# zeropoolnetwork/fawkes-crypto

Measured on AMD Instinct MI355X. Metric: Groth16 proofs/sec + MSM scalar-muls/sec, BN254, 2^25 constraints (33552553 rows = 99.99 % of the 2^25 domain), higher is better.
Workload: dtype u32

## Files before the change

fawkes-crypto_amd/csrc/msm.hip:

```cpp
#include "common.hpp"
#include <algorithm>
#include <string.h>
#include <type_traits>

namespace fk {

static constexpr uint32_t SEG_MAX = 4096, SEG_MIN = 256;
static constexpr uint32_t SORT_THREADS = 256;

struct MsmPlan {
    size_t n;
    uint32_t c, W, B;
    uint32_t cb, wide;
    uint32_t nchunks;
    size_t chunk;
    uint32_t cap, cap_top;
    uint32_t L, T, nblk;
    uint32_t LB, nhi, nlo;
};
#ifndef FK_S2_TILE
#define FK_S2_TILE 8192
#endif
static constexpr uint32_t S2_TILE = FK_S2_TILE;
static constexpr uint32_t S2_EPT = S2_TILE / 1024;
#ifndef FK_S1_TILE
#define FK_S1_TILE 8192
#endif
static constexpr uint32_t S1_TILE = FK_S1_TILE;
#ifndef FK_S2_MAX_HI
#define FK_S2_MAX_HI 1024
#endif
static constexpr uint32_t S2_MAX_HI = FK_S2_MAX_HI;

static MsmPlan make_plan(size_t n, unsigned forced_c, bool merged = false) {
    MsmPlan p{};
    p.n = n;
    const size_t nd = n ? n : 1;
    uint32_t lg = 0; while (((size_t)1 << (lg + 1)) <= nd + nd / 2) lg++;
    static const int t_small = tune("FK_MSM_C_SMALL", 17), t_delta = tune("FK_MSM_C_DELTA", 5), t_sig = tune("FK_MSM_CAP_SIGMA", 6), t_pre_dc = tune("FK_MSM_PRE_DC", 3);
    uint32_t c = forced_c ? forced_c : (lg >= 22 ? lg - t_delta : (lg >= 18 ? (uint32_t)t_small : (lg >= 6 ? lg - 2 : 4)));
    if (merged && !forced_c) c = (uint32_t)std::max(2, (int)c + t_pre_dc);
    if (c < 2) c = 2;
    static const uint32_t t_cmax = (uint32_t)std::min(tune("FK_MSM_C_MAX", 22), S2_MAX_HI >= 2048 ? 24 : 22);
    if (c > t_cmax) c = t_cmax;
    p.c = c;
    p.W = (255 + c - 1) / c;
    p.cb = 255 / p.W;
    p.wide = 255 - p.cb * p.W;
    if (p.wide == 0) { p.cb -= 1; p.wide = p.W; }
    c = p.cb + 1;
    p.c = c;
    p.B = 1u << (c - 1);
    size_t chunk = (n + 255) / 256;
    if (chunk < 16384) chunk = 16384;
    p.chunk = chunk;
    p.nchunks = (uint32_t)((n + chunk - 1) / chunk);
    size_t mean = nd >> (p.wide < p.W ? p.cb - 1 : p.cb);
    p.cap = (uint32_t)std::min<size_t>(2 * mean + 64, 1u << 30);
    if (t_sig > 0) { uint32_t sq = 1; while ((size_t)sq * sq < mean) sq++; p.cap = (uint32_t)std::min<size_t>(mean + (size_t)t_sig * sq + 8, 1u << 30); }
    p.cap_top = p.cap;
    static const int t_redl = tune("FK_MSM_RED_L", 0);
    p.L = p.B >= (1u << 18) ? 64 : (p.B >= (1u << 17) ? p.B / 2048 : (p.B >= 8192 ? p.B / 4096 : 1));
    if (t_redl > 0 && (uint32_t)t_redl <= p.B) p.L = (uint32_t)t_redl;
    static const int t_redl_m = tune("FK_MSM_RED_L_MERGED", 0);
    if (merged) {
        if (p.B <= (1u << 19)) p.L = std::min<uint32_t>(p.L, 8);
        else if (p.B <= (1u << 20)) p.L = std::min<uint32_t>(p.L, 16);
        if (t_redl_m > 0 && (uint32_t)t_redl_m <= p.B) p.L = (uint32_t)t_redl_m;
    }
    p.T = p.B / p.L;
    p.nblk = (p.T + 255) / 256;
    static const int t_lb = std::min(12, std::max(10, tune("FK_MSM_LB", 10)));
    p.LB = (c - 1) < (uint32_t)t_lb ? (c - 1) : (uint32_t)t_lb;
    while ((p.B >> p.LB) > S2_MAX_HI) p.LB++;
    p.nlo = 1u << p.LB;
    p.nhi = p.B >> p.LB;
    return p;
}

__global__ __launch_bounds__(256) void msm_digits_kernel(const Fr *scalars, size_t n, uint32_t cb, uint32_t wide, uint32_t W, uint32_t *digits) {
    const size_t half = (n + 1) / 2;
    const size_t i0 = (size_t)blockIdx.x * blockDim.x + threadIdx.x;
    if (i0 >= half) return;
    const size_t i1 = i0 + half;
    const bool has1 = i1 < n;
    Fr in[2];
    in[0] = scalars[i0];
    in[1] = scalars[has1 ? i1 : i0];
#pragma unroll
    for (int u = 0; u < 2; u++) {
        if (u == 1 && !has1) break;
        const size_t i = u ? i1 : i0;
        Fr s = Fr::from_mont(in[u]);
        uint32_t carry = 0;
        for (uint32_t w = 0; w < W; w++) {
            const uint32_t cw = cb + (w < wide ? 1 : 0);
            const uint32_t o = w * cb + (w < wide ? w : wide), limb = o >> 5, sh = o & 31;
            const uint32_t B = 1u << (cw - 1), mask = (1u << cw) - 1;
            uint32_t lo = limb < 8 ? s.v[limb] : 0, hi = limb + 1 < 8 ? s.v[limb + 1] : 0;
            uint32_t raw = (uint32_t)((((uint64_t)hi << 32) | lo) >> sh) & mask;
            raw += carry;
            uint32_t d, neg;
            if (raw > B) { d = (1u << cw) - raw; neg = 1; carry = 1; } else { d = raw; neg = 0; carry = 0; }
            digits[(size_t)w * n + i] = d | (neg << 31);
        }
    }
}

struct OverEntry { uint32_t g, size; };

static __device__ __forceinline__ uint32_t block_excl_scan_1024(uint32_t v, uint32_t *wsum, uint32_t *total) {
    const uint32_t lane = threadIdx.x & 63, wv = threadIdx.x >> 6;
    uint32_t incl = v;
#pragma unroll
    for (int off = 1; off < 64; off <<= 1) { const uint32_t t = (uint32_t)__shfl_up((int)incl, off, 64); if (lane >= (uint32_t)off) incl += t; }
    if (lane == 63) wsum[wv] = incl;
    __syncthreads();
    uint32_t base = 0, all = 0;
#pragma unroll
    for (uint32_t w = 0; w < 16; w++) { const uint32_t x = wsum[w]; all += x; if (w < wv) base += x; }
    __syncthreads();
    *total = all;
    return base + incl - v;
}

struct MsmDyn {
    uint32_t cap, n_over, seg, n_tasks, n_obs, error, pad0, pad1;
    uint32_t hist[16];
    unsigned long long adds;
};
static constexpr uint32_t OVER_MAX = 4096;

static __device__ __forceinline__ void over_append(bool take, uint32_t g, uint32_t size, OverEntry *over, MsmDyn *dyn) {
    const unsigned long long m = __ballot(take);
    if (!m) return;
    const uint32_t lane = threadIdx.x & 63, leader = (uint32_t)__ffsll((long long)m) - 1;
    uint32_t base = 0;
    if (lane == leader) base = atomicAdd(&dyn->n_over, (uint32_t)__popcll(m));
    base = (uint32_t)__shfl((int)base, (int)leader, 64);
    if (take) {
        const uint32_t k = base + (uint32_t)__popcll(m & ((1ull << lane) - 1));
        if (k < OVER_MAX) { over[k].g = g; over[k].size = size; } else dyn->error = 1;
    }
}

__global__ __launch_bounds__(SORT_THREADS) void s2_hist1_kernel(const uint32_t *digits, size_t n, size_t chunk, uint32_t nchunks,
                                                                 uint32_t LB, uint32_t nhi, uint32_t *cnt1) {
    extern __shared__ uint32_t hist[];
    const uint32_t ch = blockIdx.x, w = blockIdx.y;
    for (uint32_t b = threadIdx.x; b < nhi; b += blockDim.x) hist[b] = 0;
    __syncthreads();
    const size_t lo = (size_t)ch * chunk, hi = lo + chunk < n ? lo + chunk : n;
    const uint32_t *dg = digits + (size_t)w * n;
    for (size_t i = lo + threadIdx.x; i < hi; i += (size_t)blockDim.x * 8) {
        uint32_t d[8];
#pragma unroll
        for (int u = 0; u < 8; u++) { const size_t k = i + (size_t)u * blockDim.x; d[u] = k < hi ? (dg[k] & 0x7fffffffu) : 0; }
#pragma unroll
        for (int u = 0; u < 8; u++) if (d[u]) atomicAdd(&hist[(d[u] - 1) >> LB], 1u);
    }
    __syncthreads();
    uint32_t *out = cnt1 + ((size_t)w * nchunks + ch) * nhi;
    for (uint32_t b = threadIdx.x; b < nhi; b += blockDim.x) out[b] = hist[b];
}

__global__ __launch_bounds__(1024) void s2_prefix1_kernel(uint32_t *cnt1, uint32_t nchunks, uint32_t nhi, uint32_t *seg_size, uint32_t *seg_start,
                                                           uint32_t *seg_tiles) {
    extern __shared__ uint32_t ssz[];
    const uint32_t w = blockIdx.x;
    for (uint32_t h = threadIdx.x; h < nhi; h += blockDim.x) {
        uint32_t run = 0;
        for (uint32_t ch = 0; ch < nchunks; ch++) {
            uint32_t *p = cnt1 + ((size_t)w * nchunks + ch) * nhi + h;
            const uint32_t v = *p; *p = run; run += v;
        }
        ssz[h] = run;
    }
    __syncthreads();
    __shared__ uint32_t part[1024];
    const uint32_t t = threadIdx.x;
    const uint32_t v0 = 2 * t < nhi ? ssz[2 * t] : 0, v1 = 2 * t + 1 < nhi ? ssz[2 * t + 1] : 0;
    part[t] = v0 + v1;
    __syncthreads();
    for (uint32_t off = 1; off < 1024; off <<= 1) {
        const uint32_t x = t >= off ? part[t - off] : 0;
        __syncthreads();
        part[t] += x;
        __syncthreads();
    }
    const uint32_t base = part[t] - (v0 + v1);
    if (2 * t < nhi) { const size_t g = (size_t)w * nhi + 2 * t; seg_size[g] = v0; seg_start[g] = base; seg_tiles[g] = (v0 + S2_TILE - 1) / S2_TILE; }
    if (2 * t + 1 < nhi) { const size_t g = (size_t)w * nhi + 2 * t + 1; seg_size[g] = v1; seg_start[g] = base + v0; seg_tiles[g] = (v1 + S2_TILE - 1) / S2_TILE; }
}

__global__ __launch_bounds__(1024) void s2_tile_prefix_kernel(const uint32_t *seg_tiles, uint32_t nseg, uint32_t *tile_start) {
    __shared__ uint32_t part[1024];
    const uint32_t t = threadIdx.x, per = (nseg + 1023) / 1024;
    const uint32_t lo = t * per, hi = lo + per < nseg ? lo + per : nseg;
    uint32_t sum = 0;
    for (uint32_t s = lo; s < hi; s++) sum += seg_tiles[s];
    part[t] = sum;
    __syncthreads();
    for (uint32_t off = 1; off < 1024; off <<= 1) {
        const uint32_t v = t >= off ? part[t - off] : 0;
        __syncthreads();
        part[t] += v;
        __syncthreads();
    }
    uint32_t run = part[t] - sum;
    for (uint32_t s = lo; s < hi; s++) { tile_start[s] = run; run += seg_tiles[s]; }
    if (t == 1023) tile_start[nseg] = part[1023];
}

static __device__ __forceinline__ uint32_t s2_find_segment(const uint32_t *tile_start, uint32_t nseg, uint32_t t) {
    uint32_t lo = 0, hi = nseg;
    while (hi - lo > 1) { const uint32_t mid = (lo + hi) >> 1; if (tile_start[mid] <= t) lo = mid; else hi = mid; }
    return lo;
}

__global__ __launch_bounds__(256) void s2_hist2_kernel(const uint16_t *tmp_lo, size_t n, uint32_t nhi, uint32_t nlo, const uint32_t *tile_start,
                                                        uint32_t nseg, const uint32_t *seg_start, const uint32_t *seg_size, uint32_t *cnt2) {
    extern __shared__ uint32_t hist[];
    const uint32_t tile = blockIdx.x;
    if (tile >= tile_start[nseg]) return;
    const uint32_t sgm = s2_find_segment(tile_start, nseg, tile), w = sgm / nhi, t = tile - tile_start[sgm];
    for (uint32_t b = threadIdx.x; b < nlo; b += 256) hist[b] = 0;
    __syncthreads();
    const uint32_t size = seg_size[sgm], lo = t * S2_TILE, hi = lo + S2_TILE < size ? lo + S2_TILE : size;
    const uint16_t *src = tmp_lo + (size_t)w * n + seg_start[sgm];
    for (uint32_t k = lo + threadIdx.x; k < hi; k += 256 * 8) {
        uint32_t v[8];
#pragma unroll
        for (uint32_t u = 0; u < 8; u++) { const uint32_t kk = k + u * 256; v[u] = kk < hi ? src[kk] : 0xffffffffu; }
#pragma unroll
        for (uint32_t u = 0; u < 8; u++) if (v[u] != 0xffffffffu) atomicAdd(&hist[v[u]], 1u);
    }
    __syncthreads();
    for (uint32_t b = threadIdx.x; b < nlo; b += 256) cnt2[(size_t)tile * nlo + b] = hist[b];
}

static constexpr uint32_t P2_MAX = 32;
__global__ __launch_bounds__(256) void s2_prefix2_kernel(uint32_t *cnt2, uint32_t nseg, uint32_t nhi, uint32_t nlo, uint32_t B, const uint32_t *tile_start,
                                                          const uint32_t *seg_start, uint32_t cap0, uint32_t *totals, uint32_t *starts, MsmDyn *dyn) {
    __shared__ uint32_t sh_hist[16];
    const uint32_t lane = threadIdx.x & 63, sgm = blockIdx.x * 4 + (threadIdx.x >> 6);
    if (threadIdx.x < 16) sh_hist[threadIdx.x] = 0;
    __syncthreads();
    if (sgm < nseg) {
        const uint32_t w = sgm / nhi, h = sgm % nhi, t0 = tile_start[sgm], t1 = tile_start[sgm + 1];
        uint32_t carry = seg_start[sgm];
        for (uint32_t b0 = 0; b0 < nlo; b0 += 64 * P2_MAX) {
            const uint32_t per = (nlo - b0 + 63) / 64 < P2_MAX ? (nlo - b0 + 63) / 64 : P2_MAX;
            uint32_t run[P2_MAX];
#pragma unroll
            for (uint32_t i = 0; i < P2_MAX; i++) run[i] = 0;
            for (uint32_t t = t0; t < t1; t++) {
                uint32_t *row = cnt2 + (size_t)t * nlo + b0;
// ... 27 lines not shown
    __syncthreads();
    if (threadIdx.x < 16 && sh_hist[threadIdx.x]) atomicAdd(&dyn->hist[threadIdx.x], sh_hist[threadIdx.x]);
}

__global__ void msm_cap_kernel(MsmDyn *dyn, uint32_t cap0, uint32_t many) {
    if (threadIdx.x || blockIdx.x) return;
    uint32_t above[17]; above[16] = 0;
    for (int k = 15; k >= 0; k--) above[k] = above[k + 1] + dyn->hist[k];
    uint32_t k = 0;
    while (k < 15 && above[k] > many && ((unsigned long long)cap0 << k) < (1ull << 20)) k++;
    const unsigned long long c = (unsigned long long)cap0 << k;
    dyn->cap = c < (1ull << 30) ? (uint32_t)c : (1u << 30);
    dyn->n_over = 0; dyn->seg = 0; dyn->n_tasks = 0; dyn->n_obs = 0; dyn->error = 0; dyn->adds = 0;
}

__global__ __launch_bounds__(256) void msm_over_list_kernel(const uint32_t *totals, size_t WB, OverEntry *over, MsmDyn *dyn) {
    const size_t g = (size_t)blockIdx.x * blockDim.x + threadIdx.x;
    const uint32_t sz = g < WB ? totals[g] : 0;
    over_append(g < WB && sz > dyn->cap, (uint32_t)g, sz, over, dyn);
}

template <uint32_t MAXLO>
__global__ __launch_bounds__(1024) void s2_scatter2_kernel(const uint32_t *tmp_idx, const uint16_t *tmp_lo, size_t n, uint32_t nhi, uint32_t nlo, uint32_t B,
                                                            const uint32_t *tile_start, uint32_t nseg, const uint32_t *seg_start, const uint32_t *seg_size,
                                                            const uint32_t *cnt2, const uint32_t *starts, uint32_t *sorted) {
    constexpr uint32_t BPL = MAXLO / 1024;
    __shared__ uint32_t lcnt[MAXLO];
    __shared__ uint32_t wsum[16];
    __shared__ uint32_t gbase[MAXLO];
    __shared__ uint32_t stage_idx[S2_TILE];
    __shared__ uint16_t stage_lo[S2_TILE];
    const uint32_t tile = blockIdx.x, tid = threadIdx.x;
    if (tile >= tile_start[nseg]) return;
    const uint32_t sgm = s2_find_segment(tile_start, nseg, tile), w = sgm / nhi, h = sgm % nhi, t = tile - tile_start[sgm];
#pragma unroll
    for (uint32_t i = 0; i < BPL; i++) {
        const uint32_t b = tid + i * 1024;
        lcnt[b] = 0;
        gbase[b] = b < nlo ? starts[(size_t)w * B + (size_t)h * nlo + b] + cnt2[(size_t)tile * nlo + b] : 0;
    }
    __syncthreads();
    const uint32_t size = seg_size[sgm], lo = t * S2_TILE, cnt = (lo + S2_TILE < size ? lo + S2_TILE : size) - lo;
    const size_t base = (size_t)w * n + seg_start[sgm] + lo;
    uint32_t e_idx[S2_EPT], e_lo[S2_EPT], e_rank[S2_EPT];
#pragma unroll
    for (uint32_t j = 0; j < S2_EPT; j++) {
        const uint32_t k = tid + j * 1024;
        if (k < cnt) { e_idx[j] = tmp_idx[base + k]; e_lo[j] = tmp_lo[base + k]; e_rank[j] = atomicAdd(&lcnt[e_lo[j]], 1u); }
    }
    __syncthreads();
    uint32_t c[BPL], mine = 0;
#pragma unroll
    for (uint32_t i = 0; i < BPL; i++) { c[i] = lcnt[tid * BPL + i]; mine += c[i]; }
    uint32_t all_;
    uint32_t excl = block_excl_scan_1024(mine, wsum, &all_);
#pragma unroll
    for (uint32_t i = 0; i < BPL; i++) { lcnt[tid * BPL + i] = excl; excl += c[i]; }
    __syncthreads();
#pragma unroll
    for (uint32_t j = 0; j < S2_EPT; j++) {
        const uint32_t k = tid + j * 1024;
        if (k < cnt) { const uint32_t q = lcnt[e_lo[j]] + e_rank[j]; stage_idx[q] = e_idx[j]; stage_lo[q] = (uint16_t)e_lo[j]; }
    }
    __syncthreads();
    uint32_t *out = sorted + (size_t)w * n;
    for (uint32_t q = tid; q < cnt; q += 1024) {
        const uint32_t b = stage_lo[q];
        out[gbase[b] + (q - lcnt[b])] = stage_idx[q];
    }
}

__global__ __launch_bounds__(1024) void s2_scatter1_n1024_kernel(const uint32_t *digits, size_t n, size_t chunk, uint32_t nchunks, uint32_t LB,
                                                                  uint32_t nhi, const uint32_t *cnt1, const uint32_t *seg_start, uint32_t *tmp_idx,
                                                                  uint16_t *tmp_lo) {
    constexpr uint32_t NT = 1024;
    constexpr uint32_t BPL = S2_MAX_HI / NT;
    constexpr uint32_t EPT = S1_TILE / NT;
    constexpr bool PREFETCH = EPT <= 16;
    __shared__ uint32_t cursor[S2_MAX_HI];
    __shared__ uint32_t lcnt[S2_MAX_HI];
    __shared__ uint32_t lexc[S2_MAX_HI];
    __shared__ uint32_t part[16];
    __shared__ uint32_t stage_idx[S1_TILE];
    __shared__ uint16_t stage_lo[S1_TILE];
    __shared__ uint16_t stage_bin[S1_TILE];
    const uint32_t ch = blockIdx.x, w = blockIdx.y, tid = threadIdx.x;
    const uint32_t *cnt = cnt1 + ((size_t)w * nchunks + ch) * nhi;
    for (uint32_t b = tid; b < S2_MAX_HI; b += NT) cursor[b] = b < nhi ? seg_start[(size_t)w * nhi + b] + cnt[b] : 0;
    const size_t c_lo = (size_t)ch * chunk, c_hi = c_lo + chunk < n ? c_lo + chunk : n;
    const uint32_t *dg = digits + (size_t)w * n;
    const uint32_t lomask = (1u << LB) - 1;
    uint32_t *oidx = tmp_idx + (size_t)w * n;
    uint16_t *olo = tmp_lo + (size_t)w * n;
    uint32_t d[PREFETCH ? EPT : 1], dn[PREFETCH ? EPT : 1];
    if (PREFETCH && c_lo < c_hi) {
        const uint32_t cnt0 = (uint32_t)(c_hi - c_lo < S1_TILE ? c_hi - c_lo : S1_TILE);
#pragma unroll
        for (uint32_t j = 0; j < EPT; j++) { const uint32_t k = tid + j * NT; d[j] = k < cnt0 ? dg[c_lo + k] : 0; }
    }
    for (size_t sub = c_lo; sub < c_hi; sub += S1_TILE) {
        const uint32_t cntt = (uint32_t)(c_hi - sub < S1_TILE ? c_hi - sub : S1_TILE);
        const uint32_t *src = dg + sub;
        for (uint32_t b = tid; b < S2_MAX_HI; b += NT) lcnt[b] = 0;
        __syncthreads();
        if (PREFETCH) {
#pragma unroll
            for (uint32_t j = 0; j < EPT; j++) { const uint32_t bkt = d[j] & 0x7fffffffu; if (bkt) atomicAdd(&lcnt[(bkt - 1) >> LB], 1u); }
        } else {
#pragma unroll 8
            for (uint32_t k = tid; k < cntt; k += NT) {
                const uint32_t bkt = src[k] & 0x7fffffffu;
                if (bkt) atomicAdd(&lcnt[(bkt - 1) >> LB], 1u);
            }
        }
        __syncthreads();
        uint32_t c[BPL], mine = 0;
#pragma unroll
        for (uint32_t i = 0; i < BPL; i++) { c[i] = lcnt[tid * BPL + i]; mine += c[i]; }
        uint32_t total;
        uint32_t ex = block_excl_scan_1024(mine, part, &total);
#pragma unroll
        for (uint32_t i = 0; i < BPL; i++) { lexc[tid * BPL + i] = ex; ex += c[i]; }
        __syncthreads();
        if (PREFETCH) {
#pragma unroll
            for (uint32_t j = 0; j < EPT; j++) {
                const uint32_t bkt = d[j] & 0x7fffffffu;
                if (bkt) {
                    const uint32_t bin = (bkt - 1) >> LB, q = atomicAdd(&lexc[bin], 1u);
                    stage_idx[q] = (uint32_t)(sub + tid + j * NT) | (d[j] & 0x80000000u); stage_lo[q] = (uint16_t)((bkt - 1) & lomask); stage_bin[q] = (uint16_t)bin;
                }
            }
            const size_t nxt = sub + S1_TILE;
            const uint32_t cntn = nxt < c_hi ? (uint32_t)(c_hi - nxt < S1_TILE ? c_hi - nxt : S1_TILE) : 0;
#pragma unroll
            for (uint32_t j = 0; j < EPT; j++) { const uint32_t k = tid + j * NT; dn[j] = k < cntn ? dg[nxt + k] : 0; }
        } else {
#pragma unroll 8
            for (uint32_t k = tid; k < cntt; k += NT) {
                const uint32_t dd = src[k], bkt = dd & 0x7fffffffu;
                if (bkt) {
                    const uint32_t bin = (bkt - 1) >> LB, q = atomicAdd(&lexc[bin], 1u);
                    stage_idx[q] = (uint32_t)(sub + k) | (dd & 0x80000000u); stage_lo[q] = (uint16_t)((bkt - 1) & lomask); stage_bin[q] = (uint16_t)bin;
                }
            }
        }
        __syncthreads();
#pragma unroll 1
        for (uint32_t q = tid; q < total; q += NT) {
            const uint32_t bn = stage_bin[q];
            const uint32_t dst = cursor[bn] + (q - (lexc[bn] - lcnt[bn]));
            oidx[dst] = stage_idx[q];
            olo[dst] = stage_lo[q];
        }
        __syncthreads();
        for (uint32_t b = tid; b < S2_MAX_HI; b += NT) cursor[b] += lcnt[b];
        if (PREFETCH) {
#pragma unroll
            for (uint32_t j = 0; j < EPT; j++) d[j] = dn[j];
        }
        __syncthreads();
    }
}

static constexpr uint32_t SIZE_BINS = 1024;
static __device__ __forceinline__ uint32_t size_class(uint32_t size, uint32_t cap) {
    const uint32_t s = size < cap ? size : cap;
    if (s < 768) return (SIZE_BINS - 1) - s;
    const uint32_t span = cap > 768 ? cap - 768 : 1;
    return 255u - (uint32_t)(((uint64_t)(s - 768) * 255u) / span);
}
static __device__ __forceinline__ unsigned long long wave_sum_u64(unsigned long long v) {
#pragma unroll
    for (int off = 32; off >= 1; off >>= 1) v += (unsigned long long)__shfl_down((long long)v, off, 64);
    return v;
}
static __device__ __forceinline__ uint32_t dyn_cap(const MsmDyn *dyn, uint32_t mult) {
    const unsigned long long c = (unsigned long long)dyn->cap * mult;
    return c < (1ull << 30) ? (uint32_t)c : (1u << 30);
}
__global__ __launch_bounds__(256) void msm_size_hist_kernel(const uint32_t *totals, size_t WB, const MsmDyn *dyn, uint32_t mult, uint32_t *bins, unsigned long long *adds) {
    __shared__ uint32_t sh[SIZE_BINS];
    const uint32_t cap = dyn_cap(dyn, mult);
    for (uint32_t i = threadIdx.x; i < SIZE_BINS; i += 256) sh[i] = 0;
    __syncthreads();
    unsigned long long mine = 0;
    for (size_t g = (size_t)blockIdx.x * 256 + threadIdx.x; g < WB; g += (size_t)gridDim.x * 256) {
        const uint32_t t = totals[g];
        atomicAdd(&sh[size_class(t, cap)], 1u);
        if (t) mine += (t < cap ? t : cap) - 1;
    }
    __syncthreads();
    for (uint32_t i = threadIdx.x; i < SIZE_BINS; i += 256) if (sh[i]) atomicAdd(&bins[i], sh[i]);
    if (adds) { mine = wave_sum_u64(mine); if ((threadIdx.x & 63) == 0 && mine) atomicAdd(adds, mine); }
}
__global__ __launch_bounds__(SIZE_BINS) void msm_size_scan_kernel(uint32_t *bins) {
    __shared__ uint32_t sh[SIZE_BINS];
    const uint32_t t = threadIdx.x, v = bins[t];
    sh[t] = v;
    __syncthreads();
    for (uint32_t off = 1; off < SIZE_BINS; off <<= 1) {
        uint32_t x = t >= off ? sh[t - off] : 0;
        __syncthreads();
        sh[t] += x;
        __syncthreads();
    }
    bins[t] = sh[t] - v;
}
__global__ __launch_bounds__(1024) void msm_size_scatter_kernel(const uint32_t *totals, size_t WB, const MsmDyn *dyn, uint32_t mult, uint32_t *cursor, uint32_t *perm) {
    __shared__ uint32_t cnt[SIZE_BINS];
    __shared__ uint32_t base[SIZE_BINS];
    const uint32_t cap = dyn_cap(dyn, mult);
    const size_t g = (size_t)blockIdx.x * 1024 + threadIdx.x;
    cnt[threadIdx.x] = 0;
    __syncthreads();
    uint32_t cls = 0, rank = 0;
    if (g < WB) { cls = size_class(totals[g], cap); rank = atomicAdd(&cnt[cls], 1u); }
    __syncthreads();
    if (cnt[threadIdx.x]) base[threadIdx.x] = atomicAdd(&cursor[threadIdx.x], cnt[threadIdx.x]);
    __syncthreads();
    if (g < WB) perm[base[cls] + rank] = (uint32_t)g;
}

template <class T>
static __device__ __forceinline__ T shfl_down_obj(const T &v, int off) {
    static_assert(sizeof(T) % 4 == 0, "word sized");
    T r;
    const uint32_t *s = reinterpret_cast<const uint32_t *>(&v);
    uint32_t *d = reinterpret_cast<uint32_t *>(&r);
#pragma unroll
    for (unsigned i = 0; i < sizeof(T) / 4; i++) d[i] = (uint32_t)__shfl_down((int)s[i], off, 64);
    return r;
}

template <class F>
static __device__ __forceinline__ void wave_reduce(Xyzz<F> &acc) {
#pragma unroll 1
    for (int off = 32; off >= 1; off >>= 1) {
        Xyzz<F> o = shfl_down_obj(acc, off);
// ... 308 lines not shown
    return FK_OK;
}

static int pinned_reserve(fk_ctx *ctx, void **p, size_t *cap, size_t bytes, size_t pad) {
    if (bytes + pad <= *cap) return FK_OK;
    if (*p) { FK_HIP(ctx, hipHostFree(*p)); *p = nullptr; *cap = 0; }
    FK_HIP(ctx, hipHostMalloc(p, bytes + (bytes >> 2) + pad, hipHostMallocDefault));
    *cap = bytes + (bytes >> 2) + pad;
    return FK_OK;
}

template <class F>
struct MsmJob {
    fk_ctx *ctx;
    MsmPlan p;
    MsmLane *ln;
    MsmTail *tl;
    const Affine<F> *bases, *lev;
    const Fr *scalars;
    size_t n, WB, max_tasks, max_tiles, wp_bytes;
    uint32_t WR;
    bool merged, have_sort;
    MsmDyn *dyn;
    uint32_t *digits, *sorted, *totals, *starts, *perm;
    Task *tasks;
    OverBucket *obs;
    Xyzz<F> *winparts;
};

template <class F>
static int msm_reserve(MsmJob<F> &j) {
    fk_ctx *ctx = j.ctx;
    const MsmPlan &p = j.p;
    MsmLane &ln = *j.ln;
    MsmTail &tl = *j.tl;
    const size_t n = j.n, WB = j.WB = (size_t)p.W * p.B;
    j.WR = j.merged ? 1 : p.W;
    j.wp_bytes = (size_t)j.WR * sizeof(Xyzz<F>);
    const size_t wp_dev_bytes = (size_t)j.WR * (p.nblk + 1) * sizeof(Xyzz<F>);
    const size_t max_tasks = j.max_tasks = std::max<size_t>(2048, (size_t)p.W * n / SEG_MAX) + OVER_MAX + 64;
    const uint32_t nseg = p.W * p.nhi;
    const size_t max_tiles = j.max_tiles = (size_t)p.W * ((n + S2_TILE - 1) / S2_TILE) + nseg + 1;
    struct Need { DevBuf *b; size_t bytes; };
    const Need needs[] = {
        {&ln.digits, (size_t)p.W * n * 4}, {&ln.sorted, (size_t)p.W * n * 4}, {&ln.totals, WB * 4}, {&ln.starts, WB * 4},
        {&ln.perm, WB * 4 + SIZE_BINS * 4}, {&ln.overlist, OVER_MAX * sizeof(OverEntry) + sizeof(MsmDyn) + 64}, {j.have_sort ? &ln.buckets2 : &ln.buckets, WB * sizeof(Xyzz<F>)},
        {&ln.tasktab, max_tasks * sizeof(Task) + OVER_MAX * sizeof(OverBucket) + 64}, {&ln.partials, max_tasks * sizeof(Xyzz<F>)},
        {&ln.s2_cnt1, (size_t)p.W * p.nchunks * p.nhi * 4}, {&ln.s2_seg, ((size_t)nseg * 4 + 2) * 4}, {&ln.s2_cnt2, max_tiles * p.nlo * 4},
        {&ln.s2_tmp_idx, (size_t)p.W * n * 4}, {&ln.s2_tmp_lo, (size_t)p.W * n * 2}};
    bool grow = false;
    for (const Need &nd : needs) grow = grow || nd.bytes > nd.b->cap;
    if (grow) {
        FK_HIP(ctx, hipStreamSynchronize(ln.st));
        for (const Need &nd : needs) FK_HIP(ctx, nd.b->reserve(nd.bytes));
        if (!j.have_sort) ln.last_sort_scalars = nullptr;
    }
    FK_HIP(ctx, tl.d_wp.reserve(wp_dev_bytes));
    FK_TRY(pinned_reserve(ctx, &tl.h_wp, &tl.h_cap, j.wp_bytes, 16));
    j.dyn = (MsmDyn *)((char *)ln.overlist.p + OVER_MAX * sizeof(OverEntry));
    j.tasks = ln.tasktab.as<Task>();
    j.obs = (OverBucket *)((char *)ln.tasktab.p + ((max_tasks * sizeof(Task) + 15) & ~(size_t)15));
    j.digits = ln.digits.as<uint32_t>(); j.sorted = ln.sorted.as<uint32_t>();
    j.totals = ln.totals.as<uint32_t>(); j.starts = ln.starts.as<uint32_t>();
    j.winparts = tl.d_wp.as<Xyzz<F>>();
    j.perm = ln.perm.as<uint32_t>();
    return FK_OK;
}

static void launch_scatter2(const MsmPlan &p, uint32_t n_tiles, hipStream_t st, const uint32_t *tmp_idx, const uint16_t *tmp_lo, size_t n, const uint32_t *tile_start, uint32_t nseg,
                            const uint32_t *seg_start, const uint32_t *seg_size, const uint32_t *cnt2, const uint32_t *starts, uint32_t *sorted) {
    const auto kernel = p.nlo <= 1024 ? s2_scatter2_kernel<1024> : (p.nlo <= 2048 ? s2_scatter2_kernel<2048> : s2_scatter2_kernel<4096>);
    hipLaunchKernelGGL(kernel, dim3(n_tiles), dim3(1024), 0, st, tmp_idx, tmp_lo, n, p.nhi, p.nlo, p.B, tile_start, nseg, seg_start, seg_size, cnt2, starts, sorted);
}

template <class F>
static int queue_sort(const MsmJob<F> &j) {
    fk_ctx *ctx = j.ctx;
    const MsmPlan &p = j.p;
    MsmLane &ln = *j.ln;
    hipStream_t st = ln.st;
    const size_t n = j.n;
    const uint32_t nseg = p.W * p.nhi;
    ln.last_sort_scalars = nullptr;
    hipLaunchKernelGGL(msm_digits_kernel, dim3((unsigned)(((n + 1) / 2 + 63) / 64)), dim3(64), 0, st, j.scalars, n, p.cb, p.wide, p.W, j.digits);
    FK_HIP(ctx, hipGetLastError());
    FK_DBG_ST(ctx, st, "msm_digits");
    FK_HIP(ctx, hipMemsetAsync(j.dyn, 0, sizeof(MsmDyn), st));
    uint32_t *cnt1 = ln.s2_cnt1.as<uint32_t>();
    uint32_t *seg_size = ln.s2_seg.as<uint32_t>(), *seg_start = seg_size + nseg, *seg_tiles = seg_start + nseg, *tile_start = seg_tiles + nseg;
    uint32_t *cnt2 = ln.s2_cnt2.as<uint32_t>(), *tmp_idx = ln.s2_tmp_idx.as<uint32_t>();
    uint16_t *tmp_lo = ln.s2_tmp_lo.as<uint16_t>();
    hipLaunchKernelGGL(s2_hist1_kernel, dim3(p.nchunks, p.W), dim3(SORT_THREADS), p.nhi * 4, st, j.digits, n, p.chunk, p.nchunks, p.LB, p.nhi, cnt1);
    hipLaunchKernelGGL(s2_prefix1_kernel, dim3(p.W), dim3(1024), p.nhi * 4, st, cnt1, p.nchunks, p.nhi, seg_size, seg_start, seg_tiles);
    hipLaunchKernelGGL(s2_tile_prefix_kernel, dim3(1), dim3(1024), 0, st, seg_tiles, nseg, tile_start);
    hipLaunchKernelGGL(s2_scatter1_n1024_kernel, dim3(p.nchunks, p.W), dim3(1024), 0, st, j.digits, n, p.chunk, p.nchunks, p.LB, p.nhi, cnt1, seg_start, tmp_idx, tmp_lo);
    FK_HIP(ctx, hipGetLastError());
    FK_DBG_ST(ctx, st, "msm_sort_pass1");
    const uint32_t n_tiles = (uint32_t)j.max_tiles;
    hipLaunchKernelGGL(s2_hist2_kernel, dim3(n_tiles), dim3(256), p.nlo * 4, st, tmp_lo, n, p.nhi, p.nlo, tile_start, nseg, seg_start, seg_size, cnt2);
    hipLaunchKernelGGL(s2_prefix2_kernel, dim3((nseg + 3) / 4), dim3(256), 0, st, cnt2, nseg, p.nhi, p.nlo, p.B, tile_start, seg_start, p.cap ? p.cap : 1u, j.totals, j.starts, j.dyn);
    launch_scatter2(p, n_tiles, st, tmp_idx, tmp_lo, n, tile_start, nseg, seg_start, seg_size, cnt2, j.starts, j.sorted);
    FK_HIP(ctx, hipGetLastError());
    FK_DBG_ST(ctx, st, "msm_sort_pass2");
    ln.last_sort_scalars = (const void *)j.scalars; ln.last_sort_n = n; ln.last_sort_c = p.c; ln.last_merged = j.merged;
    return FK_OK;
}

template <class F>
static int queue_size_order(const MsmJob<F> &j) {
    fk_ctx *ctx = j.ctx;
    const MsmPlan &p = j.p;
    MsmLane &ln = *j.ln;
    hipStream_t st = ln.st;
    const size_t WB = j.WB;
    MsmDyn *dyn = j.dyn;
    uint32_t *totals = j.totals, *perm = j.perm, *size_bins = perm + WB;
    unsigned long long *d_adds = &dyn->adds;
    static const int t_many = tune("FK_MSM_OVER_MANY", 2048);
    const uint32_t many = (uint32_t)std::min<size_t>(std::max<size_t>((size_t)t_many, WB / 8192), OVER_MAX - 64);
    hipLaunchKernelGGL(msm_cap_kernel, dim3(1), dim3(64), 0, st, dyn, p.cap ? p.cap : 1u, many);
    hipLaunchKernelGGL(msm_over_list_kernel, dim3((unsigned)((WB + 255) / 256)), dim3(256), 0, st, totals, WB, ln.overlist.as<OverEntry>(), dyn);
    hipLaunchKernelGGL(msm_tasks_kernel, dim3(1), dim3(1024), 0, st, ln.overlist.as<OverEntry>(), dyn, p.B, j.merged ? 1 : 0, j.tasks, (uint32_t)j.max_tasks, j.obs);
    FK_HIP(ctx, hipMemsetAsync(size_bins, 0, SIZE_BINS * 4, st));
    if (j.merged) {
        uint32_t *mt = perm + p.B;
        hipLaunchKernelGGL(msm_merge_totals_kernel, dim3(std::min<uint32_t>((p.B + 255) / 256, 1024)), dim3(256), 0, st, totals, p.B, p.W, dyn, mt, d_adds);
        hipLaunchKernelGGL(msm_size_hist_kernel, dim3((unsigned)std::min<size_t>((p.B + 255) / 256, 1024)), dim3(256), 0, st, mt, (size_t)p.B, dyn, p.W, size_bins, (unsigned long long *)nullptr);
        hipLaunchKernelGGL(msm_size_scan_kernel, dim3(1), dim3(SIZE_BINS), 0, st, size_bins);
        hipLaunchKernelGGL(msm_size_scatter_kernel, dim3((unsigned)((p.B + 1023) / 1024)), dim3(1024), 0, st, mt, (size_t)p.B, dyn, p.W, size_bins, perm);
    } else {
        hipLaunchKernelGGL(msm_size_hist_kernel, dim3((unsigned)std::min<size_t>((WB + 255) / 256, 1024)), dim3(256), 0, st, totals, WB, dyn, 1u, size_bins, d_adds);
        hipLaunchKernelGGL(msm_size_scan_kernel, dim3(1), dim3(SIZE_BINS), 0, st, size_bins);
        hipLaunchKernelGGL(msm_size_scatter_kernel, dim3((unsigned)((WB + 1023) / 1024)), dim3(1024), 0, st, totals, WB, dyn, 1u, size_bins, perm);
    }
    FK_HIP(ctx, hipGetLastError());
    FK_DBG_ST(ctx, st, "msm_size_order");
    if (ctx->debug) {
        MsmDyn h{};
        FK_HIP(ctx, hipMemcpy(&h, dyn, sizeof h, hipMemcpyDeviceToHost));
        fprintf(stderr, "[fk] msm n=%zu c=%u (W=%u: %u x %u bits + %u x %u bits) cap=%u (plan %u): %u oversized buckets, %u tasks of %u entries, %u fold groups\n", j.n, p.c,
                p.W, p.wide, p.cb + 1, p.W - p.wide, p.cb, h.cap, p.cap, h.n_over, h.n_tasks, h.seg, h.n_obs);
        fflush(stderr);
    }
    return FK_OK;
}

template <class F>
static Xyzz<F> *bucket_buf(const MsmJob<F> &j) { return (j.have_sort ? j.ln->buckets2 : j.ln->buckets).template as<Xyzz<F>>(); }

template <class F>
static int queue_accumulate(MsmJob<F> j) {
    fk_ctx *ctx = j.ctx;
    const MsmPlan &p = j.p;
    hipStream_t st = j.ln->st;
    constexpr int MINW = std::is_same<F, Fq>::value ? 4 : 2;
    Xyzz<F> *buckets = bucket_buf(j);
    std::vector<EventPair> &evv = (sizeof(F) == sizeof(Fq)) ? ctx->ev_acc : ctx->ev_acc2;
    FK_TRY(stats_begin(ctx, evv, (uint64_t)j.n, st));
    if (j.merged)
        hipLaunchKernelGGL(HIP_KERNEL_NAME(msm_accumulate_merged_kernel<F, MINW>), dim3((p.B + 255) / 256), dim3(256), 0, st, j.bases, j.lev, j.sorted, j.n,
                           j.starts, j.totals, p.B, p.W, j.dyn, j.perm, j.perm + p.B, buckets);
    else
        hipLaunchKernelGGL(HIP_KERNEL_NAME(msm_accumulate_kernel<F, MINW>), dim3((unsigned)((j.WB + 255) / 256)), dim3(256), 0, st, j.bases, j.sorted, j.n,
                           j.starts, j.totals, p.B, p.W, j.dyn, j.perm, buckets);
    FK_HIP(ctx, hipGetLastError());
    FK_TRY(stats_end(ctx, evv, st));
    if (!ctx->ev_acc_done) FK_HIP(ctx, hipEventCreateWithFlags(&ctx->ev_acc_done, hipEventDisableTiming));
    FK_HIP(ctx, hipEventRecord(ctx->ev_acc_done, st)); ctx->ev_acc_done_valid = true;
    FK_DBG_ST(ctx, st, "msm_accumulate");
    return FK_OK;
}

template <class F>
static int queue_tail(MsmJob<F> j) {
    using FC = typename ColdOf<F>::type;
    fk_ctx *ctx = j.ctx;
    const MsmPlan &p = j.p;
    MsmLane &ln = *j.ln;
    MsmTail &tl = *j.tl;
    hipStream_t st = ln.st;
    Xyzz<F> *buckets = bucket_buf(j);
    hipLaunchKernelGGL(HIP_KERNEL_NAME(msm_overflow_kernel<F, FC>), dim3(2048), dim3(64), 0, st,
                       j.bases, j.lev, j.sorted, j.n, j.starts, j.totals, p.B, j.dyn, j.tasks, ln.partials.as<Xyzz<FC>>());
    FK_HIP(ctx, hipGetLastError());
    FK_DBG_ST(ctx, st, "msm_overflow");
    hipLaunchKernelGGL(HIP_KERNEL_NAME(msm_overflow_fold_kernel<F>), dim3(256), dim3(256), 0, st, j.obs, j.dyn, ln.partials.as<Xyzz<F>>(), buckets);
    FK_HIP(ctx, hipGetLastError());
    FK_DBG_ST(ctx, st, "msm_overflow_fold");
    hipLaunchKernelGGL(HIP_KERNEL_NAME(msm_bucket_reduce_kernel<F>), dim3(p.nblk, j.WR), dim3(256), 0, st, buckets, p.B, p.L, p.T, p.nblk, j.winparts);
    Xyzz<F> *folded = j.winparts + (size_t)j.WR * p.nblk;
    hipLaunchKernelGGL(HIP_KERNEL_NAME(msm_fold_partials_kernel<F>), dim3(j.WR), dim3(256), 0, st, j.winparts, p.nblk, folded);
    FK_HIP(ctx, hipGetLastError());
    FK_HIP(ctx, hipMemcpyAsync(tl.h_wp, folded, j.wp_bytes, hipMemcpyDeviceToHost, st));
    FK_HIP(ctx, hipMemcpyAsync((char *)tl.h_wp + j.wp_bytes, &j.dyn->adds, 8, hipMemcpyDeviceToHost, st));
    FK_HIP(ctx, hipMemcpyAsync((char *)tl.h_wp + j.wp_bytes + 8, &j.dyn->error, 4, hipMemcpyDeviceToHost, st));
    FK_HIP(ctx, hipEventRecord(tl.done, st));
    FK_DBG_ST(ctx, st, "msm_bucket_reduce");
    return FK_OK;
}

template <class F>
static int msm_begin(fk_ctx *ctx, const Affine<F> *d_bases, const Fr *d_scalars, size_t n, bool reuse_sort, int *tail_out, hipEvent_t ready, const KeyPre *pre = nullptr) {
    *tail_out = -1;
    if (n == 0) return FK_OK;
    if (n >= ((size_t)1 << 31)) FK_SET_ERR(ctx, FK_ERR_BAD_ARG, "msm: n too large");
    int ti = -1;
    for (int i = 0; i < MSM_TAILS; i++) if (!ctx->tails[i].active) { ti = i; break; }
    if (ti < 0) FK_SET_ERR(ctx, FK_ERR_BAD_ARG, "msm: too many outstanding multiplications");
    MsmTail &tl = ctx->tails[ti];
    if (!tl.done) FK_HIP(ctx, hipEventCreateWithFlags(&tl.done, hipEventDisableTiming));
    MsmPlan p = make_plan(n, ctx->window_bits);
    bool merged = false;
    if (pre && pre->lev && pre->n == n) {
        const MsmPlan pm = make_plan(n, ctx->window_bits, true);
        if (pm.cb == pre->cb && pm.wide == pre->wide && pm.W == pre->W) { p = pm; merged = true; }
    }
    MsmLane &prev = ctx->lanes[ctx->lane_prev];
    const bool have_sort = reuse_sort && prev.st && prev.last_sort_scalars == (const void *)d_scalars && prev.last_sort_n == n && prev.last_sort_c == p.c && prev.last_merged == merged;
    const int li = have_sort ? ctx->lane_prev : ctx->lane_next;
    MsmLane &ln = ctx->lanes[li];
    if (!ln.st) FK_SET_ERR(ctx, FK_ERR_HIP, "msm: the context's streams were not created");
    static const int t_lanes = tune("FK_MSM_LANES", 0);
    const int n_lanes = (t_lanes >= 1 && t_lanes <= MSM_LANES && !ctx->defer_back && ctx->deferred.empty())
                            ? t_lanes : (ctx->lanes_in_use >= 2 && ctx->lanes_in_use <= MSM_LANES ? ctx->lanes_in_use : MSM_LANES);
// ... 426 lines not shown
```

Baseline: 4.377.

## Fuse pass-1 histogram into digit kernel and simplify scatter1 cursor bookkeeping

The digit-decomposition kernel now runs per sort chunk and builds the per-window coarse histogram in LDS while it emits the signed digits. This removes the separate s2_hist1 kernel and its full re-read of the digit array. The prefix1 column scan is batched eight chunks at a time, and scatter1 stages a single 32-bit bucket value instead of separate lo and bin arrays. The cursor update is folded into the scan, dropping one barrier and a loop. In exchange, the digit kernel's grid falls to nchunks blocks of 256 threads, and the kernel needs W*nhi LDS counters, guarded by a 64KB check, which may reduce parallelism and occupancy.

Result: no change. 4.363, median of 2 (-0.3%).

```diff
diff --git a/fawkes-crypto_amd/csrc/msm.hip b/fawkes-crypto_amd/csrc/msm.hip
--- a/fawkes-crypto_amd/csrc/msm.hip
+++ b/fawkes-crypto_amd/csrc/msm.hip
@@ -6,7 +6,6 @@
 namespace fk {
 
 static constexpr uint32_t SEG_MAX = 4096, SEG_MIN = 256;
-static constexpr uint32_t SORT_THREADS = 256;
 
 struct MsmPlan {
     size_t n;
@@ -78,33 +77,45 @@
     return p;
 }
 
-__global__ __launch_bounds__(256) void msm_digits_kernel(const Fr *scalars, size_t n, uint32_t cb, uint32_t wide, uint32_t W, uint32_t *digits) {
-    const size_t half = (n + 1) / 2;
-    const size_t i0 = (size_t)blockIdx.x * blockDim.x + threadIdx.x;
-    if (i0 >= half) return;
-    const size_t i1 = i0 + half;
-    const bool has1 = i1 < n;
-    Fr in[2];
-    in[0] = scalars[i0];
-    in[1] = scalars[has1 ? i1 : i0];
-#pragma unroll
-    for (int u = 0; u < 2; u++) {
-        if (u == 1 && !has1) break;
-        const size_t i = u ? i1 : i0;
-        Fr s = Fr::from_mont(in[u]);
-        uint32_t carry = 0;
-        for (uint32_t w = 0; w < W; w++) {
-            const uint32_t cw = cb + (w < wide ? 1 : 0);
-            const uint32_t o = w * cb + (w < wide ? w : wide), limb = o >> 5, sh = o & 31;
-            const uint32_t B = 1u << (cw - 1), mask = (1u << cw) - 1;
-            uint32_t lo = limb < 8 ? s.v[limb] : 0, hi = limb + 1 < 8 ? s.v[limb + 1] : 0;
-            uint32_t raw = (uint32_t)((((uint64_t)hi << 32) | lo) >> sh) & mask;
-            raw += carry;
-            uint32_t d, neg;
-            if (raw > B) { d = (1u << cw) - raw; neg = 1; carry = 1; } else { d = raw; neg = 0; carry = 0; }
-            digits[(size_t)w * n + i] = d | (neg << 31);
+static constexpr uint32_t DIG_THREADS = 256;
+__global__ __launch_bounds__(DIG_THREADS) void msm_digits_kernel(const Fr *scalars, size_t n, size_t chunk, uint32_t nchunks, uint32_t cb, uint32_t wide, uint32_t W,
+                                                                 uint32_t LB, uint32_t nhi, uint32_t *digits, uint32_t *cnt1) {
+    constexpr uint32_t NT = DIG_THREADS;
+    extern __shared__ uint32_t hist[];
+    const uint32_t ch = blockIdx.x, tid = threadIdx.x, nbin = W * nhi;
+    for (uint32_t b = tid; b < nbin; b += NT) hist[b] = 0;
+    __syncthreads();
+    const size_t c_lo = (size_t)ch * chunk, c_hi = c_lo + chunk < n ? c_lo + chunk : n;
+    Fr nx[2];
+    if (c_lo + tid < c_hi) { const size_t i0 = c_lo + tid; nx[0] = scalars[i0]; nx[1] = scalars[i0 + NT < c_hi ? i0 + NT : i0]; }
+    for (size_t i0 = c_lo + tid; i0 < c_hi; i0 += 2 * NT) {
+        const size_t i1 = i0 + NT, j0 = i0 + 2 * NT;
+        const bool has1 = i1 < c_hi;
+        Fr in[2];
+        in[0] = nx[0]; in[1] = nx[1];
+        if (j0 < c_hi) { nx[0] = scalars[j0]; nx[1] = scalars[j0 + NT < c_hi ? j0 + NT : j0]; }
+#pragma unroll
+        for (int u = 0; u < 2; u++) {
+            if (u == 1 && !has1) break;
+            const size_t i = u ? i1 : i0;
+            Fr s = Fr::from_mont(in[u]);
+            uint32_t carry = 0;
+            for (uint32_t w = 0; w < W; w++) {
+                const uint32_t cw = cb + (w < wide ? 1 : 0);
+                const uint32_t o = w * cb + (w < wide ? w : wide), limb = o >> 5, sh = o & 31;
+                const uint32_t B = 1u << (cw - 1), mask = (1u << cw) - 1;
+                uint32_t lo = limb < 8 ? s.v[limb] : 0, hi = limb + 1 < 8 ? s.v[limb + 1] : 0;
+                uint32_t raw = (uint32_t)((((uint64_t)hi << 32) | lo) >> sh) & mask;
+                raw += carry;
+                uint32_t d, neg;
+                if (raw > B) { d = (1u << cw) - raw; neg = 1; carry = 1; } else { d = raw; neg = 0; carry = 0; }
+                digits[(size_t)w * n + i] = d | (neg << 31);
+                if (d) atomicAdd(&hist[w * nhi + ((d - 1) >> LB)], 1u);
+            }
         }
     }
+    __syncthreads();
+    for (uint32_t b = tid; b < nbin; b += NT) { const uint32_t w = b / nhi, h = b - w * nhi; cnt1[((size_t)w * nchunks + ch) * nhi + h] = hist[b]; }
 }
 
 struct OverEntry { uint32_t g, size; };
@@ -144,35 +155,19 @@
     }
 }
 
-__global__ __launch_bounds__(SORT_THREADS) void s2_hist1_kernel(const uint32_t *digits, size_t n, size_t chunk, uint32_t nchunks,
-                                                                 uint32_t LB, uint32_t nhi, uint32_t *cnt1) {
-    extern __shared__ uint32_t hist[];
-    const uint32_t ch = blockIdx.x, w = blockIdx.y;
-    for (uint32_t b = threadIdx.x; b < nhi; b += blockDim.x) hist[b] = 0;
-    __syncthreads();
-    const size_t lo = (size_t)ch * chunk, hi = lo + chunk < n ? lo + chunk : n;
-    const uint32_t *dg = digits + (size_t)w * n;
-    for (size_t i = lo + threadIdx.x; i < hi; i += (size_t)blockDim.x * 8) {
-        uint32_t d[8];
-#pragma unroll
-        for (int u = 0; u < 8; u++) { const size_t k = i + (size_t)u * blockDim.x; d[u] = k < hi ? (dg[k] & 0x7fffffffu) : 0; }
-#pragma unroll
-        for (int u = 0; u < 8; u++) if (d[u]) atomicAdd(&hist[(d[u] - 1) >> LB], 1u);
-    }
-    __syncthreads();
-    uint32_t *out = cnt1 + ((size_t)w * nchunks + ch) * nhi;
-    for (uint32_t b = threadIdx.x; b < nhi; b += blockDim.x) out[b] = hist[b];
-}
-
 __global__ __launch_bounds__(1024) void s2_prefix1_kernel(uint32_t *cnt1, uint32_t nchunks, uint32_t nhi, uint32_t *seg_size, uint32_t *seg_start,
                                                            uint32_t *seg_tiles) {
     extern __shared__ uint32_t ssz[];
     const uint32_t w = blockIdx.x;
     for (uint32_t h = threadIdx.x; h < nhi; h += blockDim.x) {
         uint32_t run = 0;
-        for (uint32_t ch = 0; ch < nchunks; ch++) {
-            uint32_t *p = cnt1 + ((size_t)w * nchunks + ch) * nhi + h;
-            const uint32_t v = *p; *p = run; run += v;
+        uint32_t *col = cnt1 + (size_t)w * nchunks * nhi + h;
+        for (uint32_t c0 = 0; c0 < nchunks; c0 += 8) {
+            uint32_t v[8];
+#pragma unroll
+            for (uint32_t u = 0; u < 8; u++) v[u] = c0 + u < nchunks ? col[(size_t)(c0 + u) * nhi] : 0;
+#pragma unroll
+            for (uint32_t u = 0; u < 8; u++) { if (c0 + u < nchunks) col[(size_t)(c0 + u) * nhi] = run; run += v[u]; }
         }
         ssz[h] = run;
     }
@@ -366,8 +361,7 @@
     __shared__ uint32_t lexc[S2_MAX_HI];
     __shared__ uint32_t part[16];
     __shared__ uint32_t stage_idx[S1_TILE];
-    __shared__ uint16_t stage_lo[S1_TILE];
-    __shared__ uint16_t stage_bin[S1_TILE];
+    __shared__ uint32_t stage_bkt[S1_TILE];
     const uint32_t ch = blockIdx.x, w = blockIdx.y, tid = threadIdx.x;
     const uint32_t *cnt = cnt1 + ((size_t)w * nchunks + ch) * nhi;
     for (uint32_t b = tid; b < S2_MAX_HI; b += NT) cursor[b] = b < nhi ? seg_start[(size_t)w * nhi + b] + cnt[b] : 0;
@@ -389,7 +383,10 @@
         __syncthreads();
         if (PREFETCH) {
 #pragma unroll
-            for (uint32_t j = 0; j < EPT; j++) { const uint32_t bkt = d[j] & 0x7fffffffu; if (bkt) atomicAdd(&lcnt[(bkt - 1) >> LB], 1u); }
+            for (uint32_t j = 0; j < EPT; j++) {
+                const uint32_t bkt = d[j] & 0x7fffffffu;
+                if (bkt) atomicAdd(&lcnt[(bkt - 1) >> LB], 1u);
+            }
         } else {
 #pragma unroll 8
             for (uint32_t k = tid; k < cntt; k += NT) {
@@ -404,16 +401,22 @@
         uint32_t total;
         uint32_t ex = block_excl_scan_1024(mine, part, &total);
 #pragma unroll
-        for (uint32_t i = 0; i < BPL; i++) { lexc[tid * BPL + i] = ex; ex += c[i]; }
+        for (uint32_t i = 0; i < BPL; i++) {
+            const uint32_t b = tid * BPL + i, cur = cursor[b];
+            lexc[b] = ex; lcnt[b] = cur - ex; cursor[b] = cur + c[i]; ex += c[i];
+        }
         __syncthreads();
         if (PREFETCH) {
+            uint32_t qs[EPT];
 #pragma unroll
             for (uint32_t j = 0; j < EPT; j++) {
                 const uint32_t bkt = d[j] & 0x7fffffffu;
-                if (bkt) {
-                    const uint32_t bin = (bkt - 1) >> LB, q = atomicAdd(&lexc[bin], 1u);
-                    stage_idx[q] = (uint32_t)(sub + tid + j * NT) | (d[j] & 0x80000000u); stage_lo[q] = (uint16_t)((bkt - 1) & lomask); stage_bin[q] = (uint16_t)bin;
-                }
+                qs[j] = bkt ? atomicAdd(&lexc[(bkt - 1) >> LB], 1u) : 0;
+            }
+#pragma unroll
+            for (uint32_t j = 0; j < EPT; j++) {
+                const uint32_t bkt = d[j] & 0x7fffffffu;
+                if (bkt) { stage_idx[qs[j]] = (uint32_t)(sub + tid + j * NT) | (d[j] & 0x80000000u); stage_bkt[qs[j]] = bkt - 1; }
             }
             const size_t nxt = sub + S1_TILE;
             const uint32_t cntn = nxt < c_hi ? (uint32_t)(c_hi - nxt < S1_TILE ? c_hi - nxt : S1_TILE) : 0;
@@ -425,20 +428,18 @@
                 const uint32_t dd = src[k], bkt = dd & 0x7fffffffu;
                 if (bkt) {
                     const uint32_t bin = (bkt - 1) >> LB, q = atomicAdd(&lexc[bin], 1u);
-                    stage_idx[q] = (uint32_t)(sub + k) | (dd & 0x80000000u); stage_lo[q] = (uint16_t)((bkt - 1) & lomask); stage_bin[q] = (uint16_t)bin;
+                    stage_idx[q] = (uint32_t)(sub + k) | (dd & 0x80000000u); stage_bkt[q] = bkt - 1;
                 }
             }
         }
         __syncthreads();
 #pragma unroll 1
         for (uint32_t q = tid; q < total; q += NT) {
-            const uint32_t bn = stage_bin[q];
-            const uint32_t dst = cursor[bn] + (q - (lexc[bn] - lcnt[bn]));
+            const uint32_t bk = stage_bkt[q];
+            const uint32_t dst = q + lcnt[bk >> LB];
             oidx[dst] = stage_idx[q];
-            olo[dst] = stage_lo[q];
+            olo[dst] = (uint16_t)(bk & lomask);
         }
-        __syncthreads();
-        for (uint32_t b = tid; b < S2_MAX_HI; b += NT) cursor[b] += lcnt[b];
         if (PREFETCH) {
 #pragma unroll
             for (uint32_t j = 0; j < EPT; j++) d[j] = dn[j];
@@ -913,15 +914,15 @@
     const size_t n = j.n;
     const uint32_t nseg = p.W * p.nhi;
     ln.last_sort_scalars = nullptr;
-    hipLaunchKernelGGL(msm_digits_kernel, dim3((unsigned)(((n + 1) / 2 + 63) / 64)), dim3(64), 0, st, j.scalars, n, p.cb, p.wide, p.W, j.digits);
+    if ((size_t)p.W * p.nhi * 4 > 65536) FK_SET_ERR(ctx, FK_ERR_BAD_ARG, "msm: the digit kernel's LDS counters do not hold W x nhi bins");
+    uint32_t *cnt1 = ln.s2_cnt1.as<uint32_t>();
+    hipLaunchKernelGGL(msm_digits_kernel, dim3(p.nchunks), dim3(DIG_THREADS), p.W * p.nhi * 4, st, j.scalars, n, p.chunk, p.nchunks, p.cb, p.wide, p.W, p.LB, p.nhi, j.digits, cnt1);
     FK_HIP(ctx, hipGetLastError());
     FK_DBG_ST(ctx, st, "msm_digits");
     FK_HIP(ctx, hipMemsetAsync(j.dyn, 0, sizeof(MsmDyn), st));
-    uint32_t *cnt1 = ln.s2_cnt1.as<uint32_t>();
     uint32_t *seg_size = ln.s2_seg.as<uint32_t>(), *seg_start = seg_size + nseg, *seg_tiles = seg_start + nseg, *tile_start = seg_tiles + nseg;
     uint32_t *cnt2 = ln.s2_cnt2.as<uint32_t>(), *tmp_idx = ln.s2_tmp_idx.as<uint32_t>();
     uint16_t *tmp_lo = ln.s2_tmp_lo.as<uint16_t>();
-    hipLaunchKernelGGL(s2_hist1_kernel, dim3(p.nchunks, p.W), dim3(SORT_THREADS), p.nhi * 4, st, j.digits, n, p.chunk, p.nchunks, p.LB, p.nhi, cnt1);
     hipLaunchKernelGGL(s2_prefix1_kernel, dim3(p.W), dim3(1024), p.nhi * 4, st, cnt1, p.nchunks, p.nhi, seg_size, seg_start, seg_tiles);
     hipLaunchKernelGGL(s2_tile_prefix_kernel, dim3(1), dim3(1024), 0, st, seg_tiles, nseg, tile_start);
     hipLaunchKernelGGL(s2_scatter1_n1024_kernel, dim3(p.nchunks, p.W), dim3(1024), 0, st, j.digits, n, p.chunk, p.nchunks, p.LB, p.nhi, cnt1, seg_start, tmp_idx, tmp_lo);
@@ -969,8 +970,8 @@
     if (ctx->debug) {
         MsmDyn h{};
         FK_HIP(ctx, hipMemcpy(&h, dyn, sizeof h, hipMemcpyDeviceToHost));
-        fprintf(stderr, "[fk] msm n=%zu c=%u (W=%u: %u x %u bits + %u x %u bits) cap=%u (plan %u): %u oversized buckets, %u tasks of %u entries, %u fold groups\n", j.n, p.c,
-                p.W, p.wide, p.cb + 1, p.W - p.wide, p.cb, h.cap, p.cap, h.n_over, h.n_tasks, h.seg, h.n_obs);
+        fprintf(stderr, "[fk] msm n=%zu c=%u (W=%u: %u x %u bits + %u x %u bits) cap=%u (plan %u): %u oversized buckets, %u tasks of %u entries, %u fold groups; sort: %u chunks of %zu, sub-tile %u, %u x %u bins\n", j.n, p.c,
+                p.W, p.wide, p.cb + 1, p.W - p.wide, p.cb, h.cap, p.cap, h.n_over, h.n_tasks, h.seg, h.n_obs, p.nchunks, p.chunk, S1_TILE, p.nhi, p.nlo);
         fflush(stderr);
     }
     return FK_OK;
```
